# steineggerlab/folddisco

Measured on AMD Instinct MI355X. Metric: structures/sec indexed, higher is better.
Workload: dtype f32+u32; 1 GPU; Swiss-Prot scale: 542000 synthetic AFDB-shaped structures (175035960 residues, 17705019118 postings, 26085150307 value bytes) index build, PDBTrRosetta default; 1 rank(s), contiguous id ranges, per rank 1 build call(s) of <= 542000 structures: one resident index, no merge; structures=542000, structures_per_gpu=542000, residues=175035960, postings=17705019118, parallelism=shard-by-structure x1, build_calls_per_rank=1

## Files before the change

### folddisco_amd/csrc/k_hash.hip

```cpp
#include "fd_device.h"
#include "fd_geom_other.h"
#ifndef FD_EMIT_WAVES
#define FD_EMIT_WAVES 5
#endif
#define FD_MSD_BUCKETS 40u

__global__ __launch_bounds__(FD_WAVE) void k_pair_count(fd_batch_view B, fd_hash_consts C, uint32_t *__restrict__ counts) {
    uint32_t w = fd_xcd_remap(blockIdx.x, B.n_work);
    if (w >= B.n_work) return;
    const uint32_t s = B.wi_struct[w];
    const uint32_t r0 = B.res_off[s], r1 = B.res_off[s + 1];
    const uint32_t i = B.wi_i0[w] + threadIdx.x;
    const bool vi = i < r1 && B.hash_ok[i];
    fd_v3 cai = {0.f, 0.f, 0.f};
    if (vi) cai = fd_load3(B.ca_xyz, i);
    uint32_t cnt = 0;
    for (uint32_t j = r0; j < r1; ++j) {
        if (!B.hash_ok[j]) continue;
        fd_v3 caj = fd_load3(B.ca_xyz, j);
        float d2 = fd_dist2(cai, caj);
        cnt += (vi && i != j && !(d2 > C.d2_max)) ? 1u : 0u;
    }
    for (int off = 32; off > 0; off >>= 1) cnt += __shfl_down(cnt, off, FD_WAVE);
    if (threadIdx.x == 0 && cnt) atomicAdd(&counts[s], cnt);
}

template <bool WRITE_IDS>
__device__ __forceinline__ void drain(const fd_batch_view &B, const fd_hash_consts &C, const uint32_t *q, uint32_t n,
                                      uint32_t i0, uint32_t r0, uint32_t s, uint32_t id, const uint64_t *seg_off,
                                      uint32_t *cursor, uint32_t *keys, uint32_t *ids) {
    const uint32_t lane = threadIdx.x;
    uint32_t base = 0;
    if (lane == 0) base = atomicAdd(&cursor[s], n);
    base = __shfl(base, 0, FD_WAVE);
    if (lane < n) {
        uint32_t e = q[lane];
        uint32_t i = i0 + (e >> 16), j = r0 + (e & 0xffffu);
        fd_v3 n1 = fd_load3(B.n_xyz, i), ca1 = fd_load3(B.ca_xyz, i), cb1 = fd_load3(B.cb_xyz, i);
        fd_v3 n2 = fd_load3(B.n_xyz, j), ca2 = fd_load3(B.ca_xyz, j), cb2 = fd_load3(B.cb_xyz, j);
        fd_feature f = fd_pair_feature(n1, ca1, cb1, n2, ca2, cb2);
        uint32_t h = fd_hash_enc(B.aa[i], B.aa[j], f, C.q);
        uint64_t pos = seg_off[s] + base + lane;
        keys[pos] = h;
        if (WRITE_IDS) ids[pos] = id;
    }
}

template <bool WRITE_IDS>
__global__ __launch_bounds__(FD_WAVE) void k_pair_emit(fd_batch_view B, fd_hash_consts C, const uint64_t *__restrict__ seg_off,
                                                       uint32_t *__restrict__ cursor, uint32_t *__restrict__ keys,
                                                       uint32_t *__restrict__ ids, uint32_t first_id) {
    __shared__ uint32_t q[2 * FD_WAVE];
    uint32_t w = fd_xcd_remap(blockIdx.x, B.n_work);
    if (w >= B.n_work) return;
    const uint32_t s = B.wi_struct[w];
    const uint32_t r0 = B.res_off[s], r1 = B.res_off[s + 1];
    const uint32_t i0 = B.wi_i0[w];
    const uint32_t lane = threadIdx.x;
    const uint32_t i = i0 + lane;
    const bool vi = i < r1 && B.hash_ok[i];
    fd_v3 cai = {0.f, 0.f, 0.f};
    if (vi) cai = fd_load3(B.ca_xyz, i);
    uint32_t qn = 0;
    for (uint32_t j = r0; j < r1; ++j) {
        if (!B.hash_ok[j]) continue;
        fd_v3 caj = fd_load3(B.ca_xyz, j);
        float d2 = fd_dist2(cai, caj);
        bool pass = vi && i != j && !(d2 > C.d2_max);
        uint64_t m = __ballot(pass);
        if (m == 0) continue;
        if (pass) q[qn + fd_mbcnt(m)] = (lane << 16) | (j - r0);
        qn += (uint32_t)__popcll(m);
        if (qn >= FD_WAVE) {
            __syncthreads();
            qn -= FD_WAVE;
            drain<WRITE_IDS>(B, C, q + qn, FD_WAVE, i0, r0, s, first_id + s, seg_off, cursor, keys, ids);
            __syncthreads();
        }
    }
    if (qn) {
        __syncthreads();
        drain<WRITE_IDS>(B, C, q, qn, i0, r0, s, first_id + s, seg_off, cursor, keys, ids);
    }
}

__global__ __launch_bounds__(256) void k_frames(fd_batch_view B, uint32_t n_res, fd_frame *__restrict__ frames) {
    uint32_t r = blockIdx.x * blockDim.x + threadIdx.x;
    if (r >= n_res) return;
    fd_frame F;
    if (B.hash_ok[r]) F = fd_make_frame(fd_load3(B.n_xyz, r), fd_load3(B.ca_xyz, r), fd_load3(B.cb_xyz, r));
    else { F = fd_frame{}; F.ca = fd_load3(B.ca_xyz, r); }
    F.pad = __uint_as_float((uint32_t)B.aa[r]);
    frames[r] = F;
}

typedef float fd_f2 __attribute__((ext_vector_type(2)));
#define FD_NOT_HASHABLE 0x100u

__device__ __forceinline__ bool fd_lane_of(uint64_t m) { return __builtin_amdgcn_inverse_ballot_w64(m); }

template <bool TYPES, class Step, class RunEnd>
__device__ __forceinline__ void fd_filter_block(const fd_batch_view &B, float d2_max, const fd_v3 &cai, uint64_t vim, uint32_t i0, uint32_t jb, uint32_t r1,
                                                float *s_cj, Step &&step, RunEnd &&run_end) {
    const uint32_t lane = threadIdx.x;
    const uint32_t jl = jb + lane;
    fd_v3 cj = {0.f, 0.f, 0.f};
    uint32_t kind = FD_NOT_HASHABLE;
    if (jl < r1) {
        cj = fd_load3(B.ca_xyz, jl);
        if (B.hash_ok[jl]) kind = TYPES ? (uint32_t)B.aa[jl] : 0u;
    }
    fd_wave_lds_fence();
    s_cj[lane] = cj.x; s_cj[FD_WAVE + lane] = cj.y; s_cj[2 * FD_WAVE + lane] = cj.z;
    fd_wave_lds_fence();
    const uint64_t okm = __ballot(kind != FD_NOT_HASHABLE);
    const uint64_t starts = __ballot(kind != (uint32_t)__shfl_up((int)kind, 1, FD_WAVE)) | 1ull;
    const bool last_block = jb + FD_WAVE >= r1;
    const uint32_t nk = okm ? 64u - (uint32_t)__builtin_clzll(okm) : 0u;
    const uint32_t nkf = (last_block && nk == 0) ? 1u : nk;
    const bool first = jb == i0;
    const fd_f2 ax = {cai.x, cai.x}, ay = {cai.y, cai.y}, az = {cai.z, cai.z};
    uint32_t k = 0;
    while (k < nkf) {
        const uint32_t t = (uint32_t)__builtin_amdgcn_readlane((int)kind, (int)k);
        const uint64_t rest = (starts >> k) >> 1;
        uint32_t ke = rest ? k + 1u + (uint32_t)__builtin_ctzll(rest) : (uint32_t)FD_WAVE;
        ke = ke < nkf ? ke : nkf;
        const bool run_last = last_block && ke >= nkf;
        const bool dead = t == FD_NOT_HASHABLE;
        if (dead && !run_last) { k = ke; continue; }
        const uint64_t vr = dead ? 0ull : vim;
        uint64_t gt = first ? (1ull << k) - 1ull : ~0ull;
        do {
            const fd_f2 xj = {s_cj[k], s_cj[k + 1]}, yj = {s_cj[FD_WAVE + k], s_cj[FD_WAVE + k + 1]}, zj = {s_cj[2 * FD_WAVE + k], s_cj[2 * FD_WAVE + k + 1]};
            const fd_f2 dx = ax - xj, dy = ay - yj, dz = az - zj;
            const fd_f2 d2 = (dx * dx + dy * dy) + dz * dz;
            const uint64_t gt1 = gt << 1 | 1ull;
            const uint64_t m0 = __ballot(!(d2.x > d2_max)) & vr & gt;
            const uint64_t m1 = (k + 1u < ke) ? (__ballot(!(d2.y > d2_max)) & vr & gt1) : 0ull;
            gt = gt1 << 1 | 1ull;
            const uint32_t k0 = k;
            k += 2;
            step(k0, t, m0, m1, run_last && k >= ke);
        } while (k < ke);
        k = ke;
        run_end(t);
    }
}

__global__ __launch_bounds__(FD_WAVE) void k_pair_count2(fd_batch_view B, fd_hash_consts C, uint32_t *__restrict__ counts) {
    __shared__ float s_cj[3 * FD_WAVE + 1];
    uint32_t w = fd_xcd_remap(blockIdx.x, B.n_work);
    if (w >= B.n_work) return;
    const uint32_t s = B.wi_struct[w];
    const uint32_t r1 = B.res_off[s + 1];
    const uint32_t i0 = B.wi_i0[w];
    const uint32_t i = i0 + threadIdx.x;
    const bool vi = i < r1 && B.hash_ok[i];
    fd_v3 cai = {0.f, 0.f, 0.f};
    if (vi) cai = fd_load3(B.ca_xyz, i);
    const uint64_t vim = __ballot(vi);
    uint32_t cnt = 0;
    for (uint32_t jb = i0; jb < r1; jb += FD_WAVE)
        fd_filter_block<false>(B, C.d2_max, cai, vim, i0, jb, r1, s_cj,
                               [&](uint32_t, uint32_t, uint64_t m0, uint64_t m1, bool) { cnt += (fd_lane_of(m0) ? 1u : 0u) + (fd_lane_of(m1) ? 1u : 0u); },
                               [](uint32_t) {});
    cnt *= 2u;
    for (int off = 32; off > 0; off >>= 1) cnt += __shfl_down(cnt, off, FD_WAVE);
    if (threadIdx.x == 0 && cnt) atomicAdd(&counts[s], cnt);
}

__global__ __launch_bounds__(256) void k_frames_perm(fd_batch_view B, fd_frame *__restrict__ frames, float *__restrict__ ca_perm, uint8_t *__restrict__ ok_perm,
                                                     uint8_t *__restrict__ aa_perm, unsigned long long *__restrict__ wide_flag) {
    __shared__ uint32_t cnt[32], cur[32];
    const uint32_t s = blockIdx.x;
    const uint32_t r0 = B.res_off[s], r1 = B.res_off[s + 1];
    if (threadIdx.x < 32) cnt[threadIdx.x] = 0;
    __syncthreads();
    for (uint32_t r = r0 + threadIdx.x; r < r1; r += 256) {
        const uint32_t a = B.aa[r];
        atomicAdd(&cnt[(B.hash_ok[r] && a < 20u) ? a : 20u], 1u);
    }
    __syncthreads();
    if (threadIdx.x == 0) { uint32_t run = 0; for (int k = 0; k < 21; ++k) { cur[k] = run; run += cnt[k]; } }
    __syncthreads();
    for (uint32_t r = r0 + threadIdx.x; r < r1; r += 256) {
        const uint32_t a = B.aa[r];
        bool ok = B.hash_ok[r] != 0;
        if (ok && a >= 20u) {
            ok = false;
            if (wide_flag) atomicOr(wide_flag, 1ull);
        }
        const uint32_t p = r0 + atomicAdd(&cur[(ok && a < 20u) ? a : 20u], 1u);
        fd_frame F;
        const fd_v3 ca = fd_load3(B.ca_xyz, r);
        if (ok) F = fd_make_frame(fd_load3(B.n_xyz, r), ca, fd_load3(B.cb_xyz, r));
        else { F = fd_frame{}; F.ca = ca; }
        F.pad = __uint_as_float(a);
        frames[p] = F;
        ca_perm[3ull * p] = ca.x; ca_perm[3ull * p + 1] = ca.y; ca_perm[3ull * p + 2] = ca.z;
        ok_perm[p] = ok ? 1 : 0;
        aa_perm[p] = (uint8_t)a;
    }
}

__global__ __launch_bounds__(FD_WAVE) void k_pair_count_msd(fd_batch_view B, fd_hash_consts C, uint32_t *__restrict__ counts) {
    __shared__ uint32_t s_cnt[FD_WAVE];
    __shared__ float s_cj[3 * FD_WAVE + 1];
    uint32_t w = fd_xcd_remap(blockIdx.x, B.n_work);
    if (w >= B.n_work) return;
    const uint32_t s = B.wi_struct[w];
    const uint32_t r1 = B.res_off[s + 1];
    const uint32_t i0 = B.wi_i0[w];
    const uint32_t lane = threadIdx.x;
    const uint32_t i = i0 + lane;
    const bool vi = i < r1 && B.hash_ok[i];
    fd_v3 cai = {0.f, 0.f, 0.f};
    uint32_t aai = 0;
    if (vi) { cai = fd_load3(B.ca_xyz, i); aai = B.aa[i]; }
    s_cnt[lane] = 0;
    __syncthreads();
    const uint64_t vim = __ballot(vi);
    uint32_t c_lo = 0, c_hi = 0, run = 0;
    const uint32_t hi_i = aai >> 4;
    for (uint32_t jb = i0; jb < r1; jb += FD_WAVE)
        fd_filter_block<true>(B, C.d2_max, cai, vim, i0, jb, r1, s_cj,
                              [&](uint32_t, uint32_t, uint64_t m0, uint64_t m1, bool) { run += (fd_lane_of(m0) ? 1u : 0u) + (fd_lane_of(m1) ? 1u : 0u); },
                              [&](uint32_t t) {
                                  if (t >= 16u) c_hi += run; else c_lo += run;
                                  if (run) atomicAdd(&s_cnt[(t * 2u + hi_i) & (FD_WAVE - 1u)], run);
                                  run = 0;
                              });
    if (c_lo) atomicAdd(&s_cnt[aai * 2u], c_lo);
    if (c_hi) atomicAdd(&s_cnt[aai * 2u + 1u], c_hi);
    __syncthreads();
    if (lane < FD_MSD_BUCKETS && s_cnt[lane]) atomicAdd(&counts[(uint64_t)lane * B.n_struct + s], s_cnt[lane]);
}

__device__ __forceinline__ fd_frame load_frame(const fd_frame *__restrict__ frames, uint32_t r) {
    const float4 *p = reinterpret_cast<const float4 *>(frames + r);
    float4 a = p[0], b = p[1], c = p[2], d = p[3], e = p[4];
    fd_frame F;
    F.ca = {a.x, a.y, a.z}; F.cb = {a.w, b.x, b.y}; F.r1 = {b.z, b.w, c.x}; F.t1 = {c.y, c.z, c.w};
    F.len = d.x; F.pad = d.y; F.s2 = {d.z, d.w, e.x}; F.nv2 = {e.y, e.z, e.w};
    return F;
}
__device__ __forceinline__ fd_frame hot_frame(const float4 &a, const float4 &b, const float4 &c, const float4 &d) {
    fd_frame F{};
    F.ca = {a.x, a.y, a.z}; F.cb = {a.w, b.x, b.y}; F.r1 = {b.z, b.w, c.x}; F.t1 = {c.y, c.z, c.w};
    F.len = d.x; F.pad = d.y;
    return F;
}

__device__ __attribute__((noinline)) uint2 pair_both_tab_exact(const fd_frame *__restrict__ frames, uint32_t i, uint32_t j, uint32_t aai,
                                                               uint32_t aaj, float dist_disc, float ang_disc, const uint32_t *tab) {
    fd_frame Fi = load_frame(frames, i), Fj = load_frame(frames, j);
    fd_quant q;
    q.dist_disc = dist_disc; q.ang_disc = ang_disc; q.ang2_disc = 0.0f; q.type = FD_HASH_PDBTR;
    uint32_t a, b;
    fd_pair_both_tab(Fi, Fj, aai, aaj, q, tab, &a, &b);
    return make_uint2(a, b);
}

template <int TAB, bool IDS16, bool MSD, bool DT = false>
__device__ __forceinline__ void drain2(const fd_batch_view &B, const fd_frame *__restrict__ frames, const fd_hash_consts &C,
                                       const uint32_t *tab, const uint32_t *q, uint32_t n, uint32_t i0, uint32_t r0, uint32_t s, uint32_t id,
                                       const uint64_t *seg_off, uint32_t *cursor, uint32_t *keys, void *ids, const float4 *s_fi,
                                       uint32_t *s_bc, uint64_t *s_bb, const uint64_t *s_boff) {
    const uint32_t lane = threadIdx.x;
    uint32_t base = 0, gb = 0, slots = 0;
    if (!MSD) {
        if (lane == 0) base = atomicAdd(&cursor[s], 2u * n);
        base = __shfl(base, 0, FD_WAVE);
    } else {
        s_bc[lane] = 0;
        fd_wave_lds_fence();
        if (lane < n) {
            const uint32_t e = q[lane], il = (e >> 16) & 63u, aj = e >> 22;
            const uint32_t ai = TAB == 2 ? __float_as_uint(s_fi[192 + il].y) : (uint32_t)B.aa[i0 + il];
            const uint32_t bf = ai * 2u + (aj >> 4), br = aj * 2u + (ai >> 4);
            slots = atomicAdd(&s_bc[bf], 1u) | atomicAdd(&s_bc[br], 1u) << 8 | bf << 16 | br << 24;
        }
        fd_wave_lds_fence();
        if (lane < FD_MSD_BUCKETS) { const uint32_t c = s_bc[lane]; if (c) gb = atomicAdd(&cursor[(uint64_t)lane * B.n_struct + s], c); }
    }
    uint32_t h_ij = 0, h_ji = 0, aai = 0, aaj = 0;
    if (lane < n) {
        uint32_t e = q[lane];
        uint32_t i = i0 + ((e >> 16) & 63u), j = r0 + (e & 0xffffu);
        if (TAB == 2) {
            const uint32_t il = (e >> 16) & 63u;
            const fd_frame Fi = hot_frame(s_fi[il], s_fi[64 + il], s_fi[128 + il], s_fi[192 + il]);
            const float4 *pj = reinterpret_cast<const float4 *>(frames + j);
            const fd_frame Fj = hot_frame(pj[0], pj[1], pj[2], pj[3]);
            aai = __float_as_uint(Fi.pad); aaj = __float_as_uint(Fj.pad);
#if defined(FD_EMIT_STUB) && FD_EMIT_STUB == 1
            h_ij = aai << 25 | aaj << 20 | (__float_as_uint(Fj.ca.x) & 0xfffffu); h_ji = aaj << 25 | aai << 20 | (__float_as_uint(Fi.ca.x) & 0xfffffu);
            if (false)
#endif
            if (!fd_pair_both_spec<DT>(Fi, Fj, aai, aaj, C.q, tab, tab + 32, &h_ij, &h_ji, tab + 64)) {
                uint2 h = pair_both_tab_exact(frames, i, j, B.aa[i], B.aa[j], C.q.dist_disc, C.q.ang_disc, tab);
                h_ij = h.x; h_ji = h.y;
                if (C.spec_miss) atomicAdd(C.spec_miss, 1ull);
            }
        } else if (TAB == 1) {
            uint2 h = pair_both_tab_exact(frames, i, j, B.aa[i], B.aa[j], C.q.dist_disc, C.q.ang_disc, tab);
            h_ij = h.x; h_ji = h.y;
        } else {
            fd_frame Fi = load_frame(frames, i), Fj = load_frame(frames, j);
            fd_pair_both(Fi, Fj, B.aa[i], B.aa[j], C.q, &h_ij, &h_ji);
        }
    }
    if (MSD) {
        asm volatile("" : "+v"(gb));
        if (lane < FD_MSD_BUCKETS) s_bb[lane] = s_boff[lane] + gb;
        fd_wave_lds_fence();
        if (lane < n) {
            const uint32_t sf = slots & 255u, sr = (slots >> 8) & 255u, bf = (slots >> 16) & 255u, br = slots >> 24;
            if ((((h_ij | h_ji) >> 30) || (h_ij >> 24) != bf || (h_ji >> 24) != br) && C.wide_flag) atomicOr(C.wide_flag, 1ull);
            const uint64_t pf = s_bb[bf] + sf, pr = s_bb[br] + sr;
            keys[pf] = (h_ij << 24) | s;
            keys[pr] = (h_ji << 24) | s;
            ((uint16_t *)ids)[pf] = (uint16_t)(h_ij >> 8);
            ((uint16_t *)ids)[pr] = (uint16_t)(h_ji >> 8);
        }
        return;
    }
    if (lane < n) {
        const uint64_t so = seg_off[s];
        uint64_t pos = so * C.seg_mul + (uint64_t)C.seg_cfg * (seg_off[s + 1] - so) + base + lane;
        if (IDS16) {
            if (((h_ij | h_ji) >> 30) && C.wide_flag) atomicOr(C.wide_flag, 1ull);
            uint32_t hi = s >> 16;
            uint16_t lo = (uint16_t)(s & 0xffffu);
            keys[pos] = (h_ij << 2) | hi;
            keys[pos + n] = (h_ji << 2) | hi;
            ((uint16_t *)ids)[pos] = lo;
            ((uint16_t *)ids)[pos + n] = lo;
        } else {
            keys[pos] = h_ij;
            keys[pos + n] = h_ji;
            ((uint32_t *)ids)[pos] = id;
            ((uint32_t *)ids)[pos + n] = id;
        }
    }
}

template <int TAB, bool IDS16, bool MSD, bool DT = false>
__global__ __launch_bounds__(FD_WAVE, FD_EMIT_WAVES) void k_pair_emit2(fd_batch_view B, const fd_frame *__restrict__ frames, fd_hash_consts C,
                                                        const uint64_t *__restrict__ seg_off, uint32_t *__restrict__ cursor,
                                                        uint32_t *__restrict__ keys, void *__restrict__ ids, uint32_t first_id) {
    __shared__ uint32_t q[3 * FD_WAVE];
    __shared__ float s_cj[3 * FD_WAVE + 1];
    __shared__ uint32_t tab[DT ? 64 + FD_DIST_NTHR + 1 : 64];
    uint32_t w = fd_xcd_remap(blockIdx.x, B.n_work);
    if (w >= B.n_work) return;
    if (TAB) {
        if (DT && threadIdx.x < FD_DIST_NTHR) tab[64 + threadIdx.x] = fd_dist_thr_bits[threadIdx.x];
        if (threadIdx.x == 0) {
            fd_fill_bintab(tab);
            for (int k = 0; k < FD_BINTAB_WORDS; ++k) tab[32 + k] = tab[k];
            for (int m = 0; m < 4; ++m)
                for (int k = 0; k < 4; ++k) { uint32_t v = tab[32 + 7 + 5 * m + k]; tab[32 + 7 + 5 * m + k] = v > 0x7f7fffffu ? 0x7f7fffffu : v; }
        }
        __syncthreads();
    }
    const uint32_t s = B.wi_struct[w];
    const uint32_t r0 = B.res_off[s], r1 = B.res_off[s + 1];
    const uint32_t i0 = B.wi_i0[w];
    const uint32_t lane = threadIdx.x;
    const uint32_t i = i0 + lane;
    const bool vi = i < r1 && B.hash_ok[i];
    fd_v3 cai = {0.f, 0.f, 0.f};
    if (vi) cai = fd_load3(B.ca_xyz, i);
    __shared__ float4 s_fi[4 * FD_WAVE];
    if (TAB == 2 && i < r1) {
        const float4 *fp = reinterpret_cast<const float4 *>(frames + i);
#pragma unroll
        for (int k = 0; k < 4; ++k) s_fi[k * FD_WAVE + lane] = fp[k];
    }
    __shared__ uint32_t s_bc[MSD ? FD_WAVE : 1];
    __shared__ uint64_t s_bb[MSD ? FD_MSD_BUCKETS : 1], s_boff[MSD ? FD_MSD_BUCKETS : 1];
    if (MSD && lane < FD_MSD_BUCKETS) s_boff[lane] = seg_off[(uint64_t)lane * B.n_struct + s];
    __syncthreads();
    const uint64_t vim = __ballot(vi);
    const uint32_t lane16 = lane << 16;
    uint32_t qn = 0;
    for (uint32_t jb = i0; jb < r1; jb += FD_WAVE) {
        const uint32_t jrel = jb - r0;
        fd_filter_block<MSD>(B, C.d2_max, cai, vim, i0, jb, r1, s_cj,
            [&](uint32_t k, uint32_t t, uint64_t m0, uint64_t m1, bool last) {
                const uint32_t tag = (MSD ? t << 22 : 0u) | (jrel + k);
                if (m0) {
                    if (fd_lane_of(m0)) q[__builtin_amdgcn_mbcnt_hi((uint32_t)(m0 >> 32), __builtin_amdgcn_mbcnt_lo((uint32_t)m0, qn))] = lane16 | tag;
                    qn += (uint32_t)__popcll(m0);
                }
                if (m1) {
                    if (fd_lane_of(m1)) q[__builtin_amdgcn_mbcnt_hi((uint32_t)(m1 >> 32), __builtin_amdgcn_mbcnt_lo((uint32_t)m1, qn))] = lane16 | (tag + 1u);
                    qn += (uint32_t)__popcll(m1);
                }
                while (qn >= FD_WAVE || (last && qn)) {
                    fd_wave_lds_fence();
                    uint32_t n = qn < FD_WAVE ? qn : FD_WAVE;
                    qn -= n;
                    drain2<TAB, IDS16, MSD, DT>(B, frames, C, tab, q + qn, n, i0, r0, s, first_id + s, seg_off, cursor, keys, ids, s_fi, s_bc, s_bb, s_boff);
                    fd_wave_lds_fence();
                }
            },
            [](uint32_t) {});
    }
}

__global__ __launch_bounds__(FD_WAVE) void k_row_count(fd_batch_view B, fd_hash_consts C, uint32_t *__restrict__ row_cnt, float cutoff) {
    uint32_t w = fd_xcd_remap(blockIdx.x, B.n_work);
    if (w >= B.n_work) return;
    const uint32_t s = B.wi_struct[w];
    const uint32_t r0 = B.res_off[s], r1 = B.res_off[s + 1];
    const uint32_t i = B.wi_i0[w] + threadIdx.x;
    if (i >= r1) return;
    if (fd_own_descriptor(C.q.type)) {
        uint32_t cnt = 0;
        if (B.aa[i] != 255)
            for (uint32_t j = r0; j < r1; ++j)
                cnt += (j != i && B.aa[j] != 255 && fd_accept_other(C.q.type, B, r0, r1, i, j, cutoff)) ? 1u : 0u;
        row_cnt[i] = cnt;
        return;
    }
    const bool vi = B.hash_ok[i];
    fd_v3 cai = fd_load3(B.ca_xyz, i);
    uint32_t cnt = 0;
    for (uint32_t j = r0; j < r1; ++j) {
        if (!B.hash_ok[j]) continue;
        float d2 = fd_dist2(cai, fd_load3(B.ca_xyz, j));
        cnt += (vi && i != j && !(d2 > C.d2_max)) ? 1u : 0u;
    }
    row_cnt[i] = cnt;
}

__global__ __launch_bounds__(FD_WAVE) void k_row_emit(fd_batch_view B, fd_hash_consts C, const uint64_t *__restrict__ row_off,
                                                      uint32_t *__restrict__ keys, float cutoff, uint32_t *__restrict__ ids, uint32_t first_id, int ids_partner) {
    uint32_t w = fd_xcd_remap(blockIdx.x, B.n_work);
    if (w >= B.n_work) return;
    const uint32_t s = B.wi_struct[w];
    const uint32_t r0 = B.res_off[s], r1 = B.res_off[s + 1];
    const uint32_t i = B.wi_i0[w] + threadIdx.x;
    if (i >= r1) return;
    if (fd_own_descriptor(C.q.type)) {
        if (B.aa[i] == 255) return;
        uint64_t pos = row_off[i];
        float f[FD_NFEAT];
        for (uint32_t j = r0; j < r1; ++j) {
            if (j == i || B.aa[j] == 255 || !fd_feature_other(C.q.type, B, r0, r1, i, j, cutoff, f)) continue;
            if (ids) ids[pos] = ids_partner ? j : first_id + s;
            keys[pos++] = fd_hash_other(C.q.type, f, C.q);
        }
        return;
    }
    if (!B.hash_ok[i]) return;
    fd_v3 n1 = fd_load3(B.n_xyz, i), ca1 = fd_load3(B.ca_xyz, i), cb1 = fd_load3(B.cb_xyz, i);
    uint32_t aa1 = B.aa[i];
    uint64_t pos = row_off[i];
    for (uint32_t j = r0; j < r1; ++j) {
        if (!B.hash_ok[j] || i == j) continue;
        fd_v3 ca2 = fd_load3(B.ca_xyz, j);
        if (fd_dist2(ca1, ca2) > C.d2_max) continue;
        fd_v3 n2 = fd_load3(B.n_xyz, j), cb2 = fd_load3(B.cb_xyz, j);
        fd_feature f = fd_pair_feature(n1, ca1, cb1, n2, ca2, cb2);
        if (ids) ids[pos] = ids_partner ? j : first_id + s;
        keys[pos++] = fd_hash_enc(aa1, B.aa[j], f, C.q);
    }
}

__global__ void k_hash_ok(const uint8_t *__restrict__ aa, const uint8_t *__restrict__ cb_valid, uint8_t *__restrict__ ok, uint64_t n) {
    uint64_t k = (uint64_t)blockIdx.x * blockDim.x + threadIdx.x;
    if (k < n) ok[k] = (aa[k] != 255 && (cb_valid == nullptr || cb_valid[k])) ? 1 : 0;
}

__global__ void k_selfcheck(fd_quant q, uint32_t *__restrict__ out ) {
    if (threadIdx.x != 0 || blockIdx.x != 0) return;
    const fd_v3 N[3] = {{6.661f, 8.291f, 43.860f}, {10.483f, 7.756f, 49.260f}, {5.260f, -1.068f, 41.296f}};
    const fd_v3 CA[3] = {{6.994f, 8.354f, 42.405f}, {9.429f, 7.479f, 48.266f}, {5.547f, 0.158f, 42.050f}};
    const fd_v3 CB[3] = {{8.251f, 7.488f, 42.026f}, {10.033f, 6.489f, 47.255f}, {5.773f, 1.360f, 41.130f}};
    const uint32_t AA[3] = {8u, 3u, 15u};
    const int PI[6] = {1, 1, 0, 0, 2, 2}, PJ[6] = {0, 2, 1, 2, 1, 0};
    uint32_t tab[64 + FD_DIST_NTHR + 1];
    fd_fill_bintab(tab);
    for (int k = 0; k < FD_BINTAB_WORDS; ++k) tab[32 + k] = tab[k];
    for (int m = 0; m < 4; ++m)
        for (int k = 0; k < 4; ++k) { uint32_t v = tab[32 + 7 + 5 * m + k]; tab[32 + 7 + 5 * m + k] = v > 0x7f7fffffu ? 0x7f7fffffu : v; }
    for (int k = 0; k < FD_DIST_NTHR; ++k) tab[64 + k] = fd_dist_thr_bits[k];
    fd_frame F[3];
    for (int r = 0; r < 3; ++r) F[r] = fd_make_frame(N[r], CA[r], CB[r]);
    for (int k = 0; k < 6; ++k) {
        const int i = PI[k], j = PJ[k];
        out[k] = fd_hash_pdbtr(AA[i], AA[j], fd_pair_feature(N[i], CA[i], CB[i], N[j], CA[j], CB[j]), q);
        uint32_t a, b;
        fd_pair_both_tab(F[i], F[j], AA[i], AA[j], q, tab, &a, &b);
        out[6 + k] = a;
        if (!fd_pair_both_spec(F[i], F[j], AA[i], AA[j], q, tab, tab + 32, &a, &b)) fd_pair_both_tab(F[i], F[j], AA[i], AA[j], q, tab, &a, &b);
        out[12 + k] = a;
        if (!fd_pair_both_spec<true>(F[i], F[j], AA[i], AA[j], q, tab, tab + 32, &a, &b, tab + 64)) fd_pair_both_tab(F[i], F[j], AA[i], AA[j], q, tab, &a, &b);
        out[18 + k] = a;
    }
}

extern "C++" {
void fd_launch_selfcheck(const fd_quant &q, uint32_t *out, hipStream_t st) { hipLaunchKernelGGL(k_selfcheck, dim3(1), dim3(64), 0, st, q, out); }
void fd_launch_hash_ok(const uint8_t *aa, const uint8_t *cb_valid, uint8_t *ok, uint64_t n, hipStream_t st) {
    if (!n) return;
    hipLaunchKernelGGL(k_hash_ok, dim3((unsigned)((n + 255) / 256)), dim3(256), 0, st, aa, cb_valid, ok, n);
}
static inline unsigned grid_for(uint32_t n_work) { return ((n_work + 7u) / 8u) * 8u; }
void fd_launch_pair_count(const fd_batch_view &B, const fd_hash_consts &C, uint32_t *counts, hipStream_t st) {
    if (!B.n_work) return;
    hipLaunchKernelGGL(k_pair_count, dim3(grid_for(B.n_work)), dim3(FD_WAVE), 0, st, B, C, counts);
}
void fd_launch_pair_emit(const fd_batch_view &B, const fd_hash_consts &C, const uint64_t *seg_off, uint32_t *cursor,
                         uint32_t *keys, uint32_t *ids, uint32_t first_id, hipStream_t st) {
    if (!B.n_work) return;
    if (ids)
        hipLaunchKernelGGL(k_pair_emit<true>, dim3(grid_for(B.n_work)), dim3(FD_WAVE), 0, st, B, C, seg_off, cursor, keys, ids, first_id);
    else
        hipLaunchKernelGGL(k_pair_emit<false>, dim3(grid_for(B.n_work)), dim3(FD_WAVE), 0, st, B, C, seg_off, cursor, keys, ids, first_id);
}
void fd_launch_frames(const fd_batch_view &B, uint64_t n_res, void *frames, hipStream_t st) {
    if (!n_res) return;
    hipLaunchKernelGGL(k_frames, dim3((unsigned)((n_res + 255) / 256)), dim3(256), 0, st, B, (uint32_t)n_res, (fd_frame *)frames);
}
void fd_launch_pair_count2(const fd_batch_view &B, const fd_hash_consts &C, uint32_t *counts, hipStream_t st) {
    if (!B.n_work) return;
    hipLaunchKernelGGL(k_pair_count2, dim3(grid_for(B.n_work)), dim3(FD_WAVE), 0, st, B, C, counts);
}
void fd_launch_pair_emit2(const fd_batch_view &B, const void *frames, const fd_hash_consts &C, const uint64_t *seg_off, uint32_t *cursor,
                          uint32_t *keys, void *ids, bool ids16, uint32_t first_id, hipStream_t st) {
    if (!B.n_work) return;
    dim3 g(grid_for(B.n_work)), b(FD_WAVE);
    const fd_frame *F = (const fd_frame *)frames;
    if (C.use_tab >= 2 && ids16) hipLaunchKernelGGL((k_pair_emit2<2, true, false>), g, b, 0, st, B, F, C, seg_off, cursor, keys, ids, first_id);
    else if (C.use_tab >= 2) hipLaunchKernelGGL((k_pair_emit2<2, false, false>), g, b, 0, st, B, F, C, seg_off, cursor, keys, ids, first_id);
    else if (C.use_tab && ids16) hipLaunchKernelGGL((k_pair_emit2<1, true, false>), g, b, 0, st, B, F, C, seg_off, cursor, keys, ids, first_id);
    else if (C.use_tab) hipLaunchKernelGGL((k_pair_emit2<1, false, false>), g, b, 0, st, B, F, C, seg_off, cursor, keys, ids, first_id);
    else if (ids16) hipLaunchKernelGGL((k_pair_emit2<0, true, false>), g, b, 0, st, B, F, C, seg_off, cursor, keys, ids, first_id);
    else hipLaunchKernelGGL((k_pair_emit2<0, false, false>), g, b, 0, st, B, F, C, seg_off, cursor, keys, ids, first_id);
}
void fd_launch_frames_perm(const fd_batch_view &B, void *frames, float *ca_perm, uint8_t *ok_perm, uint8_t *aa_perm, unsigned long long *wide_flag, hipStream_t st) {
    if (!B.n_struct) return;
    hipLaunchKernelGGL(k_frames_perm, dim3(B.n_struct), dim3(256), 0, st, B, (fd_frame *)frames, ca_perm, ok_perm, aa_perm, wide_flag);
}
void fd_launch_pair_count_msd(const fd_batch_view &B, const fd_hash_consts &C, uint32_t *counts, hipStream_t st) {
    if (!B.n_work) return;
    hipLaunchKernelGGL(k_pair_count_msd, dim3(grid_for(B.n_work)), dim3(FD_WAVE), 0, st, B, C, counts);
}
void fd_launch_pair_emit_msd(const fd_batch_view &B, const void *frames, const fd_hash_consts &C, const uint64_t *seg_off, uint32_t *cursor, uint32_t *keys,
                             uint16_t *ids, hipStream_t st) {
    if (!B.n_work) return;
    dim3 g(grid_for(B.n_work)), b(FD_WAVE);
    const fd_frame *F = (const fd_frame *)frames;
    if (C.use_tab == 3) hipLaunchKernelGGL((k_pair_emit2<2, true, true, true>), g, b, 0, st, B, F, C, seg_off, cursor, keys, (void *)ids, 0u);
    else if (C.use_tab == 2) hipLaunchKernelGGL((k_pair_emit2<2, true, true>), g, b, 0, st, B, F, C, seg_off, cursor, keys, (void *)ids, 0u);
    else if (C.use_tab) hipLaunchKernelGGL((k_pair_emit2<1, true, true>), g, b, 0, st, B, F, C, seg_off, cursor, keys, (void *)ids, 0u);
    else hipLaunchKernelGGL((k_pair_emit2<0, true, true>), g, b, 0, st, B, F, C, seg_off, cursor, keys, (void *)ids, 0u);
}
void fd_launch_row_count(const fd_batch_view &B, const fd_hash_consts &C, uint32_t *row_cnt, float cutoff, hipStream_t st) {
    if (!B.n_work) return;
    hipLaunchKernelGGL(k_row_count, dim3(grid_for(B.n_work)), dim3(FD_WAVE), 0, st, B, C, row_cnt, cutoff);
}
void fd_launch_row_emit(const fd_batch_view &B, const fd_hash_consts &C, const uint64_t *row_off, uint32_t *keys, float cutoff, uint32_t *ids,
                        uint32_t first_id, hipStream_t st, int ids_partner) {
    if (!B.n_work) return;
    hipLaunchKernelGGL(k_row_emit, dim3(grid_for(B.n_work)), dim3(FD_WAVE), 0, st, B, C, row_off, keys, cutoff, ids, first_id, ids_partner);
}
}
```

Before: 1.599 million structures/s.

## Restructure pair-count kernels with prefetched partner loads and 4-wide LDS scan

Result: no change. 1.613 million structures/s, median of 6 (+0.9%).

```diff
diff --git a/folddisco_amd/csrc/k_hash.hip b/folddisco_amd/csrc/k_hash.hip
--- a/folddisco_amd/csrc/k_hash.hip
+++ b/folddisco_amd/csrc/k_hash.hip
@@ -95,9 +95,16 @@
 }
 
 typedef float fd_f2 __attribute__((ext_vector_type(2)));
+typedef float fd_f4 __attribute__((ext_vector_type(4)));
 #define FD_NOT_HASHABLE 0x100u
 
 __device__ __forceinline__ bool fd_lane_of(uint64_t m) { return __builtin_amdgcn_inverse_ballot_w64(m); }
+
+__device__ __forceinline__ fd_f2 fd_pair_d2(const fd_f2 ax, const fd_f2 ay, const fd_f2 az, const fd_f2 xj, const fd_f2 yj, const fd_f2 zj) {
+    const fd_f2 dx = ax - xj, dy = ay - yj, dz = az - zj;
+    return (dx * dx + dy * dy) + dz * dz;
+}
+__device__ __forceinline__ bool fd_pair_near(float d2, float d2_max) { return !(d2 > d2_max); }
 
 template <bool TYPES, class Step, class RunEnd>
 __device__ __forceinline__ void fd_filter_block(const fd_batch_view &B, float d2_max, const fd_v3 &cai, uint64_t vim, uint32_t i0, uint32_t jb, uint32_t r1,
@@ -133,11 +140,10 @@
         uint64_t gt = first ? (1ull << k) - 1ull : ~0ull;
         do {
             const fd_f2 xj = {s_cj[k], s_cj[k + 1]}, yj = {s_cj[FD_WAVE + k], s_cj[FD_WAVE + k + 1]}, zj = {s_cj[2 * FD_WAVE + k], s_cj[2 * FD_WAVE + k + 1]};
-            const fd_f2 dx = ax - xj, dy = ay - yj, dz = az - zj;
-            const fd_f2 d2 = (dx * dx + dy * dy) + dz * dz;
+            const fd_f2 d2 = fd_pair_d2(ax, ay, az, xj, yj, zj);
             const uint64_t gt1 = gt << 1 | 1ull;
-            const uint64_t m0 = __ballot(!(d2.x > d2_max)) & vr & gt;
-            const uint64_t m1 = (k + 1u < ke) ? (__ballot(!(d2.y > d2_max)) & vr & gt1) : 0ull;
+            const uint64_t m0 = __ballot(fd_pair_near(d2.x, d2_max)) & vr & gt;
+            const uint64_t m1 = (k + 1u < ke) ? (__ballot(fd_pair_near(d2.y, d2_max)) & vr & gt1) : 0ull;
             gt = gt1 << 1 | 1ull;
             const uint32_t k0 = k;
             k += 2;
@@ -148,23 +154,79 @@
     }
 }
 
+struct fd_partner { fd_v3 ca; uint32_t ok, aa; };
+__device__ __forceinline__ uint32_t fd_kind(const fd_partner &P) { return P.ok ? P.aa : FD_NOT_HASHABLE; }
+
+template <bool TYPES>
+__device__ __forceinline__ fd_partner fd_load_partner(const fd_batch_view &B, uint32_t jl, uint32_t r1) {
+    fd_partner P = {{0.f, 0.f, 0.f}, 0u, 0u};
+    if (jl < r1) {
+        P.ca = fd_load3(B.ca_xyz, jl);
+        P.ok = B.hash_ok[jl];
+        if (TYPES) P.aa = B.aa[jl];
+    }
+    return P;
+}
+
+template <bool FIRST, class RunEnd>
+__device__ __forceinline__ void fd_count_block(uint32_t kind, float d2_max, const fd_f2 ax, const fd_f2 ay, const fd_f2 az, const float *s_cj, RunEnd &&run_end) {
+    const uint32_t lane = threadIdx.x;
+    const uint64_t okm = __ballot(kind != FD_NOT_HASHABLE);
+    const uint64_t starts = __ballot(kind != (uint32_t)__shfl_up((int)kind, 1, FD_WAVE)) | 1ull;
+    const uint32_t nk = okm ? 64u - (uint32_t)__builtin_clzll(okm) : 0u;
+    uint32_t t = FD_NOT_HASHABLE, run = 0;
+    for (uint32_t k4 = 0; k4 < nk; k4 += 4u) {
+        const uint32_t sb = (uint32_t)(starts >> k4) & 0xfu;
+        if (sb == 0u && t == FD_NOT_HASHABLE) continue;
+        const fd_f4 xj = *reinterpret_cast<const fd_f4 *>(s_cj + k4), yj = *reinterpret_cast<const fd_f4 *>(s_cj + FD_WAVE + k4),
+                    zj = *reinterpret_cast<const fd_f4 *>(s_cj + 2 * FD_WAVE + k4);
+        const fd_f2 da = fd_pair_d2(ax, ay, az, xj.xy, yj.xy, zj.xy), db = fd_pair_d2(ax, ay, az, xj.zw, yj.zw, zj.zw);
+        const float d2[4] = {da.x, da.y, db.x, db.y};
+        if (sb == 0u) {
+#pragma unroll
+            for (uint32_t p = 0; p < 4u; ++p) run += (fd_pair_near(d2[p], d2_max) && (!FIRST || k4 + p > lane)) ? 1u : 0u;
+        } else {
+#pragma unroll
+            for (uint32_t p = 0; p < 4u; ++p) {
+                if ((sb >> p) & 1u) {
+                    if (t != FD_NOT_HASHABLE) run_end(t, run);
+                    run = 0;
+                    t = (uint32_t)__builtin_amdgcn_readlane((int)kind, (int)(k4 + p));
+                }
+                run += (fd_pair_near(d2[p], d2_max) && (!FIRST || k4 + p > lane)) ? 1u : 0u;
+            }
+        }
+    }
+    if (t != FD_NOT_HASHABLE) run_end(t, run);
+}
+
+template <bool TYPES, class RunEnd>
+__device__ __forceinline__ void fd_count_item(const fd_batch_view &B, float d2_max, const fd_partner &self, uint32_t i0, uint32_t r1, float *s_cj, RunEnd &&run_end) {
+    const uint32_t lane = threadIdx.x;
+    const fd_f2 ax = {self.ca.x, self.ca.x}, ay = {self.ca.y, self.ca.y}, az = {self.ca.z, self.ca.z};
+    fd_partner P = self;
+    for (uint32_t jb = i0; jb < r1; jb += FD_WAVE) {
+        fd_wave_lds_fence();
+        s_cj[lane] = P.ca.x; s_cj[FD_WAVE + lane] = P.ca.y; s_cj[2 * FD_WAVE + lane] = P.ca.z;
+        fd_wave_lds_fence();
+        const uint32_t kind = fd_kind(P);
+        if (jb + FD_WAVE < r1) P = fd_load_partner<TYPES>(B, jb + FD_WAVE + lane, r1);
+        if (jb == i0) fd_count_block<true>(kind, d2_max, ax, ay, az, s_cj, run_end);
+        else fd_count_block<false>(kind, d2_max, ax, ay, az, s_cj, run_end);
+    }
+}
+
 __global__ __launch_bounds__(FD_WAVE) void k_pair_count2(fd_batch_view B, fd_hash_consts C, uint32_t *__restrict__ counts) {
-    __shared__ float s_cj[3 * FD_WAVE + 1];
+    __shared__ __attribute__((aligned(16))) float s_cj[3 * FD_WAVE];
     uint32_t w = fd_xcd_remap(blockIdx.x, B.n_work);
     if (w >= B.n_work) return;
     const uint32_t s = B.wi_struct[w];
     const uint32_t r1 = B.res_off[s + 1];
     const uint32_t i0 = B.wi_i0[w];
-    const uint32_t i = i0 + threadIdx.x;
-    const bool vi = i < r1 && B.hash_ok[i];
-    fd_v3 cai = {0.f, 0.f, 0.f};
-    if (vi) cai = fd_load3(B.ca_xyz, i);
-    const uint64_t vim = __ballot(vi);
+    const fd_partner self = fd_load_partner<false>(B, i0 + threadIdx.x, r1);
+    const bool vi = self.ok != 0;
     uint32_t cnt = 0;
-    for (uint32_t jb = i0; jb < r1; jb += FD_WAVE)
-        fd_filter_block<false>(B, C.d2_max, cai, vim, i0, jb, r1, s_cj,
-                               [&](uint32_t, uint32_t, uint64_t m0, uint64_t m1, bool) { cnt += (fd_lane_of(m0) ? 1u : 0u) + (fd_lane_of(m1) ? 1u : 0u); },
-                               [](uint32_t) {});
+    fd_count_item<false>(B, C.d2_max, self, i0, r1, s_cj, [&](uint32_t, uint32_t run) { cnt += vi ? run : 0u; });
     cnt *= 2u;
     for (int off = 32; off > 0; off >>= 1) cnt += __shfl_down(cnt, off, FD_WAVE);
     if (threadIdx.x == 0 && cnt) atomicAdd(&counts[s], cnt);
@@ -206,31 +268,26 @@
 
 __global__ __launch_bounds__(FD_WAVE) void k_pair_count_msd(fd_batch_view B, fd_hash_consts C, uint32_t *__restrict__ counts) {
     __shared__ uint32_t s_cnt[FD_WAVE];
-    __shared__ float s_cj[3 * FD_WAVE + 1];
+    __shared__ __attribute__((aligned(16))) float s_cj[3 * FD_WAVE];
     uint32_t w = fd_xcd_remap(blockIdx.x, B.n_work);
     if (w >= B.n_work) return;
     const uint32_t s = B.wi_struct[w];
     const uint32_t r1 = B.res_off[s + 1];
     const uint32_t i0 = B.wi_i0[w];
     const uint32_t lane = threadIdx.x;
-    const uint32_t i = i0 + lane;
-    const bool vi = i < r1 && B.hash_ok[i];
-    fd_v3 cai = {0.f, 0.f, 0.f};
-    uint32_t aai = 0;
-    if (vi) { cai = fd_load3(B.ca_xyz, i); aai = B.aa[i]; }
+    const fd_partner self = fd_load_partner<true>(B, i0 + lane, r1);
+    const bool vi = self.ok != 0;
+    const uint32_t aai = vi ? self.aa : 0u;
     s_cnt[lane] = 0;
     __syncthreads();
-    const uint64_t vim = __ballot(vi);
-    uint32_t c_lo = 0, c_hi = 0, run = 0;
+    uint32_t c_lo = 0, c_hi = 0;
     const uint32_t hi_i = aai >> 4;
-    for (uint32_t jb = i0; jb < r1; jb += FD_WAVE)
-        fd_filter_block<true>(B, C.d2_max, cai, vim, i0, jb, r1, s_cj,
-                              [&](uint32_t, uint32_t, uint64_t m0, uint64_t m1, bool) { run += (fd_lane_of(m0) ? 1u : 0u) + (fd_lane_of(m1) ? 1u : 0u); },
-                              [&](uint32_t t) {
-                                  if (t >= 16u) c_hi += run; else c_lo += run;
-                                  if (run) atomicAdd(&s_cnt[(t * 2u + hi_i) & (FD_WAVE - 1u)], run);
-                                  run = 0;
-                              });
+    fd_count_item<true>(B, C.d2_max, self, i0, r1, s_cj,
+                        [&](uint32_t t, uint32_t run) {
+                            run = vi ? run : 0u;
+                            if (t >= 16u) c_hi += run; else c_lo += run;
+                            if (run) atomicAdd(&s_cnt[(t * 2u + hi_i) & (FD_WAVE - 1u)], run);
+                        });
     if (c_lo) atomicAdd(&s_cnt[aai * 2u], c_lo);
     if (c_hi) atomicAdd(&s_cnt[aai * 2u + 1u], c_hi);
     __syncthreads();
```
